# erreur404/Motion-generation-using-quadratic-programs

Hardware: AMD Instinct MI355X
Metric: QP solves/sec at n=7,p=6,m=14 batch=65536; achieved HBM GB/s vs peak (higher is better)
Workload: dtype f64; 1 GPU; C1: 65536 x (n=7, p=6, m=14) general QPs per GPU; kind=general, n=7, p=6, m=14, batch_per_gpu=65536, global_batch=65536, kernel=qp_lane<N=7,M=14>, layout=qp_major, arithmetic=exact: the reference's operation order, bitwise, streams=3, input_sets=5, cold_inputs=True, parallelism=batch-sharded x1

## Files before the change

### motion-generation-using-quadratic-programs_amd/csrc/qp_lane.hip

```cpp
#include <type_traits>
#include <utility>

#include "qp_common.h"

#ifndef QPGPU_LANE_FAST
#define QPGPU_LANE_FAST 0
#endif
#ifndef QPGPU_LANE_UNALIGNED
#define QPGPU_LANE_UNALIGNED 0
#endif
#ifndef QPGPU_LANE_UNIT
#define QPGPU_LANE_UNIT 0
#endif
#if QPGPU_LANE_UNIT && QPGPU_LANE_FAST
#error "the unit-Hessian lane kernels restate the reference's operation order only"
#endif
#if QPGPU_LANE_UNIT && QPGPU_LANE_UNALIGNED
#define QPK_LANE_NS qpk_unit_u
#define QP_LANE_KERNEL qp_lane_unit_kernel
#define QPK_LANE_C(name) name##_unit_u
#elif QPGPU_LANE_UNIT
#define QPK_LANE_NS qpk_unit
#define QP_LANE_KERNEL qp_lane_unit_kernel
#define QPK_LANE_C(name) name##_unit
#elif QPGPU_LANE_FAST && QPGPU_LANE_UNALIGNED
#define QPK_LANE_NS qpk_fast_u
#define QP_LANE_KERNEL qp_lane_fast_kernel
#define QPK_LANE_C(name) name##_fast_u
#elif QPGPU_LANE_FAST
#define QPK_LANE_NS qpk_fast
#define QP_LANE_KERNEL qp_lane_fast_kernel
#define QPK_LANE_C(name) name##_fast
#elif QPGPU_LANE_UNALIGNED
#define QPK_LANE_NS qpk_u
#define QP_LANE_KERNEL qp_lane_kernel
#define QPK_LANE_C(name) name##_u
#else
#define QPK_LANE_NS qpk
#define QP_LANE_KERNEL qp_lane_kernel
#define QPK_LANE_C(name) name
#endif

#ifndef QPGPU_LANE_STAMPS
#define QPGPU_LANE_STAMPS 1
#endif
#if defined(QPGPU_LANE_OCC2) || defined(QPGPU_LANE_DMA_P0) || defined(QPGPU_LANE_CE_LATE) ||       \
    defined(QPGPU_LANE_WARMUP) || defined(QPGPU_LANE_LOOPTOP_EXIT) || defined(QPGPU_LANE_FULL) || \
    defined(QPGPU_LANE_AB_C1ONLY) || defined(QPGPU_LANE_AB_N8P0ONLY)
#error "retired build switch: its default is folded into qp_lane.hip; the other side is an earlier revision (DESIGN 5.15, tools/ab_build.sh SRCFILE=)"
#endif

namespace QPK_LANE_NS {
using namespace qpk;
constexpr bool kFast = QPGPU_LANE_FAST != 0;
constexpr bool kStamps = QPGPU_LANE_STAMPS != 0;
__device__ __forceinline__ void lstamp(const QpArgs& a, int slot) {
  if constexpr (kStamps) qp_stamp(a, slot);
}


struct AgprD {
  uint32_t lo, hi;
};
__device__ __forceinline__ AgprD to_agpr(double v) {
  const uint64_t u = __builtin_bit_cast(uint64_t, v);
  AgprD a;
  asm("v_accvgpr_write_b32 %0, %1" : "=a"(a.lo) : "v"((uint32_t)u));
  asm("v_accvgpr_write_b32 %0, %1" : "=a"(a.hi) : "v"((uint32_t)(u >> 32)));
  return a;
}
__device__ __forceinline__ double from_agpr(const AgprD& a) {
  uint32_t lo, hi;
  asm volatile("v_accvgpr_read_b32 %0, %1" : "=v"(lo) : "a"(a.lo));
  asm volatile("v_accvgpr_read_b32 %0, %1" : "=v"(hi) : "a"(a.hi));
  return __builtin_bit_cast(double, ((uint64_t)hi << 32) | lo);
}

constexpr int kQpw = 64;
constexpr int kLaneOcc = 1;
constexpr int kStage = 5120;
constexpr int kScanDepth = 2;
using LdsD = __attribute__((address_space(3))) double;
using LdsC = __attribute__((address_space(3))) char;
using LdsV = __attribute__((address_space(3))) void;
using GlobalV = __attribute__((address_space(1))) void;
template <int... K, class F>
__device__ __forceinline__ void for_seq_impl(std::integer_sequence<int, K...>, F&& f) {
  (f(std::integral_constant<int, K>{}), ...);
}
template <int N, class F>
__device__ __forceinline__ void for_seq(F&& f) {
  for_seq_impl(std::make_integer_sequence<int, N>{}, f);
}


template <int NM, int MM, int T, bool EXACT, int PX, bool SAFE, bool DUAL = false, bool BOX = false,
          bool FULL = false>
__device__ __forceinline__ bool lane_body(const QpArgs& a, LdsD* lds) {
  double* const sbuf = (double*)lds;
  static_assert(MM <= 64, "bitmask bookkeeping holds m <= 64");
  static_assert(!BOX || (!kFast && MM == 2 * NM), "the box mode is the exact build's, m = 2n");
  static_assert(!FULL || (!kFast && !QPGPU_LANE_UNALIGNED && EXACT && PX >= 0 && !DUAL && !BOX),
                "the full-wave form is the exact aligned build's, for a compile-time shape");
  static_assert(!DUAL || (!kFast && (BOX || (!EXACT && PX < 0))),
                "the dual mode is the exact build's general instantiation, or a box form");
  using RI = RIdx<NM>;
  constexpr int STAGE = kStage;
  constexpr bool F = kFast && !SAFE;
  bool fok = true;
  constexpr bool kLanePrefetch = PX != 0 && !BOX;

  const int lane = threadIdx.x;
  const int64_t b0 = (int64_t)blockIdx.x * kQpw;
  const int64_t b = b0 + lane;
  const int valid = (int)min<int64_t>(kQpw, a.batch - b0);
  const bool live = FULL || lane < valid;

  const int n = EXACT ? NM : a.n;
  const int m = EXACT ? MM : a.m;
  const int p = PX >= 0 ? PX : a.p;
  const double inf = dinf();

#if QPGPU_LANE_UNALIGNED
  const bool full = false;
#else
  const bool full = FULL || (T == 64) || (valid == kQpw);
#endif
  auto copy_chunk = [&](auto J, const double* src, int nd, int off, int k0) {
    constexpr int j = decltype(J)::value;
    static_assert(j >= 0 && j * 1024 < 4096, "the chunk's offset is the instruction's immediate");
    const int e = k0 + 2 * lane;
    __builtin_amdgcn_global_load_lds((const GlobalV*)(e + j * 128 < nd ? src + e : src),
                                     (LdsV*)(lds + off + k0), 16, j * 1024, 0);
  };
  auto copy_run = [&](const double* src, int nd, int off, int k0) {
    copy_chunk(std::integral_constant<int, 0>{}, src, nd, off, k0);
    if (k0 + 128 < nd) copy_chunk(std::integral_constant<int, 1>{}, src, nd, off, k0);
    if (k0 + 256 < nd) copy_chunk(std::integral_constant<int, 2>{}, src, nd, off, k0);
    if (k0 + 384 < nd) copy_chunk(std::integral_constant<int, 3>{}, src, nd, off, k0);
  };
  auto copy_span = [&](const double* src, int nd, int off) {
    if constexpr (FULL) {
#pragma unroll
      for (int k0 = 0; k0 < nd; k0 += 512) copy_run(src, nd, off, k0);
    } else {
#pragma unroll 4
      for (int k = 0; k < nd; k += 128) copy_chunk(std::integral_constant<int, 0>{}, src, nd, off, k);
    }
  };
#if QPGPU_LANE_UNALIGNED
  auto stage_all = [&](const double* X, int E, int off) {
    if constexpr (T == 64) {
      const double* src = X + b0 * (int64_t)E + lane;
      for (int e = 0; e < E; e++) sbuf[off + e * kQpw + lane] = src[e * kQpw];
    } else if (live) {
      const double* src = X + b * (int64_t)E;
      for (int e = 0; e < E; e++) sbuf[off + lane * E + e] = src[e];
    }
  };
  (void)copy_span;
#else
  auto stage_all = [&](const double* X, int E, int off) {
    if (full) {
      copy_span(X + b0 * (int64_t)E, kQpw * E, off);
    } else if (live) {
      const double* src = X + b * (int64_t)E;
      for (int e = 0; e < E; e++) sbuf[off + lane * E + e] = src[e];
    }
  };
#endif
  auto rd_all = [&](int off, int E, int k) -> double {
    if constexpr (T == 64)
      return sbuf[off + k * 64 + lane];
    else
      return sbuf[off + lane * E + k];
  };
  auto view = [&](double* X, int E) -> double* {
    if constexpr (T == 64)
      return X + b0 * (int64_t)E + lane;
    else
      return X + b * (int64_t)E;
  };

  int status = QPGPU_QP_OK;
  double fval = 0.0;
  int iter = 0;
  double xv[NM];
#pragma unroll
  for (int i = 0; i < NM; i++) xv[i] = 0.0;
  double c1 = 0.0, c2 = 0.0;
  constexpr int RB = (STAGE - kQpw * NM) / 2 * 2;
  static_assert(RB >= kQpw * NM * NM, "G and g0 staging exceed the stage buffer");
  constexpr int kCiRowsFit = (RB / kQpw) / MM;
  constexpr int kCiRows = (!BOX && EXACT && T == 1 && MM % 2 == 0) ? (kCiRowsFit < NM ? kCiRowsFit : NM) : 0;
  constexpr bool kCiDma = kCiRows > 0 && PX > 0;
  constexpr int kCeN = PX > 0 ? NM * PX + PX : 1;
  [[maybe_unused]] AgprD ceag[kCiDma ? kCeN : 1];
  const bool dma = kCiDma && (FULL || (a.flags & kArgAligned16));
  double Jreg[NM][NM];
  bool ce_staged = false;
  bool ce_agpr = false;
  constexpr int kPfCI = (NM * MM * 8 + 127) / 128 + 1, kPfC0 = (MM * 8 + 127) / 128 + 1;
  [[maybe_unused]] uint32_t pf[kPfCI + kPfC0];
  bool warmed = false;
  auto warmup = [&]() {
    warmed = true;
    if (live) {
      const int off = dma ? kCiRows * MM * 8 : 0;
      const char* c = reinterpret_cast<const char*>(a.CI + b * (int64_t)(n * m)) + off;
      const char* c0 = reinterpret_cast<const char*>(a.ci0 + b * (int64_t)m);
      const int bc = n * m * 8 - off, b0c = m * 8;
#pragma unroll
      for (int k = 0; k < kPfCI; k++)
        pf[k] = (bc >= 4) ? *reinterpret_cast<const uint32_t*>(c + min(k * 128, bc - 4)) : 0u;
#pragma unroll
      for (int k = 0; k < kPfC0; k++)
        pf[kPfCI + k] = (b0c >= 4) ? *reinterpret_cast<const uint32_t*>(c0 + min(k * 128, b0c - 4)) : 0u;
    }
  };
  constexpr int kCiPieces = kCiRows * MM / 2;
  static_assert(kCiPieces * 16 <= 4096, "the piece's offset is the instruction's immediate");
  auto dma_ci_part = [&](int part, int parts) {
    const int per = (kCiPieces + parts - 1) / parts;
    const double* src = a.CI + (live ? b : b0) * (int64_t)(NM * MM);
    for_seq<kCiPieces>([&](auto K) {
      constexpr int k = decltype(K)::value;
      if (k >= part * per && k < (part + 1) * per)
        __builtin_amdgcn_global_load_lds((const GlobalV*)src, (LdsV*)((LdsC*)lds + k * (kQpw * 16 - 16)), 16,
                                         16 * k, 0);
    });
  };
  lstamp(a, 0);
  [[maybe_unused]] double bv[BOX ? MM : 1];
  if constexpr (BOX) {
    const double* hib = view(const_cast<double*>(a.hi), n);
    const double* lob = view(const_cast<double*>(a.lo), n);
#pragma unroll
    for (int v = 0; v < NM; v++) {
      const double h = (live && v < n) ? hib[v * T] : 0.0;
      const double l = (live && v < n) ? lob[v * T] : 0.0;
      bv[v] = h;
      bv[NM + v] = -l;
    }
  }

  bool chol_ok = live;
  double bad_sum = 0.0;
  {
#if !QPGPU_LANE_UNIT
    double Gr[NM][NM];
#endif
    const int offg0 = RB;
#if !QPGPU_LANE_UNIT
    stage_all(a.G, n * n, 0);
#endif
    stage_all(a.g0, n, offg0);
    __syncthreads();
    double g0v[NM];
#pragma unroll
    for (int i = 0; i < NM; i++) {
#if !QPGPU_LANE_UNIT
#pragma unroll
      for (int j = 0; j < NM; j++) {
        const double v = (i < n && j < n) ? rd_all(0, n * n, i * n + j) : 0.0;
        Gr[i][j] = live ? v : 0.0;
      }
#endif
      const double v0 = i < n ? rd_all(offg0, n, i) : 0.0;
      g0v[i] = live ? v0 : 0.0;
    }
    __syncthreads();
    lstamp(a, 9);
    const int npB = n * p;
    const int offcB = (kQpw * npB + 127) / 128 * 128;
    const bool stageB = p > 0 && offcB + kQpw * p <= STAGE;
    auto round_b = [&](int part) {
      constexpr int parts = NM;
      if (!stageB) return;
      if (!full) {
        if (part == 0) {
          stage_all(a.CE, npB, 0);
          stage_all(a.ce0, p, offcB);
        }
        return;
      }
      const double* ce = a.CE + b0 * (int64_t)npB;
      const double* c0 = a.ce0 + b0 * (int64_t)p;
      if constexpr (EXACT && PX > 0) {
        constexpr int nce = (kQpw * NM * PX + 127) / 128, tot = nce + (kQpw * PX + 127) / 128;
        constexpr int per = (tot + parts - 1) / parts;
        for_seq<tot>([&](auto C) {
          constexpr int c = decltype(C)::value;
          constexpr int arr = c < nce ? 0 : nce;
          constexpr int run = c - c % per > arr ? c - c % per : arr;
          constexpr int j = (c - run) % 4, k0 = (c - j - arr) * 128;
          if (c >= part * per && c < (part + 1) * per) {
            if constexpr (c < nce)
              copy_chunk(std::integral_constant<int, j>{}, ce, kQpw * NM * PX, 0, k0);
            else
              copy_chunk(std::integral_constant<int, j>{}, c0, kQpw * PX, nce * 128, k0);
          }
        });
      } else {
        const int nce = (kQpw * npB + 127) / 128, tot = nce + (kQpw * p + 127) / 128;
        const int per = (tot + parts - 1) / parts;
        for (int c = part * per; c < min(tot, (part + 1) * per); c++) {
          if (c < nce)
            copy_chunk(std::integral_constant<int, 0>{}, ce, kQpw * npB, 0, c * 128);
          else
            copy_chunk(std::integral_constant<int, 0>{}, c0, kQpw * p, offcB, (c - nce) * 128);
        }
      }
    };
#if QPGPU_LANE_UNIT
#pragma unroll
    for (int i = 0; i < NM; i++) {
      round_b(i);
      if (i < n) c1 += 1.0;
    }
#else
#pragma unroll
    for (int i = 0; i < NM; i++)
      if (i < n) c1 += Gr[i][i];
#pragma unroll
    for (int i = 0; i < NM; i++) {
      round_b(i);
      if (i < n && chol_ok) {
        double sum = Gr[i][i];
#pragma unroll
        for (int k = i - 1; k >= 0; k--) sum -= Gr[i][k] * Gr[i][k];
        if (sum <= 0.0) {
          chol_ok = false;
          bad_sum = sum;
        } else {
          const double dg = sqrt(sum);
          Gr[i][i] = dg;
          const double rdg = F ? frcp(dg) : 0.0;
#pragma unroll
          for (int j = i + 1; j < NM; j++)
            if (j < n) {
              double s2 = Gr[i][j];
#pragma unroll
              for (int k = i - 1; k >= 0; k--) s2 -= Gr[i][k] * Gr[j][k];
              Gr[j][i] = ldiv_r<F>(s2, dg, rdg, fok);
            }
#pragma unroll
          for (int k = i + 1; k < NM; k++) Gr[i][k] = Gr[k][i];
        }
      }
    }
    if (!FULL && (a.flags & QPGPU_FLAG_WRITE_FACTOR) && live) {
      double* Gw = view(a.G, n * n);
#pragma unroll
      for (int i = 0; i < NM; i++)
#pragma unroll
        for (int j = 0; j < NM; j++)
          if (i < n && j < n) Gw[(i * n + j) * T] = Gr[i][j];
    }
#endif
    auto land_round_b = [&]() {
    if (p > 0) {
      const int np_ = n * p;
      const int offc = (kQpw * np_ + 127) / 128 * 128;
      ce_staged = offc + kQpw * p <= STAGE;
      __syncthreads();
      lstamp(a, 10);
      if constexpr (kCiDma) {
        if (dma && ce_staged) {
#pragma unroll
          for (int e = 0; e < NM * PX; e++) {
            const double v = rd_all(0, np_, e);
            ceag[e] = to_agpr(live ? v : 0.0);
          }
#pragma unroll
          for (int e = 0; e < PX; e++) {
            const double v = rd_all(offc, p, e);
            ceag[NM * PX + e] = to_agpr(live ? v : 0.0);
          }
          ce_agpr = true;
          __syncthreads();
          lstamp(a, 11);
        }
      }
    }
    };
#if QPGPU_LANE_UNIT
    if (chol_ok) {
#pragma unroll
      for (int r = 0; r < NM; r++) {
#pragma unroll
        for (int j = 0; j < NM; j++) Jreg[r][j] = (r < n && j == r) ? 1.0 : 0.0;
        if (r < n) c2 += 1.0;
      }
#pragma unroll
      for (int i = 0; i < NM; i++) xv[i] = -g0v[i];
#pragma unroll
      for (int i = 0; i < NM; i++)
        if (i < n) fval += g0v[i] * xv[i];
      fval = 0.5 * fval;
    }
#else
    if (chol_ok) {
      bool lfin = true;
#pragma unroll
      for (int i = 0; i < NM; i++)
#pragma unroll
        for (int j = 0; j <= i; j++)
          if (i < n) lfin = lfin && (fabs(Gr[i][j]) < inf);
      double rdiag[NM];
#pragma unroll
      for (int i = 0; i < NM; i++) rdiag[i] = (F && i < n) ? frcp(Gr[i][i]) : 0.0;
      auto build_j = [&](const bool skip) {
#pragma unroll
        for (int r = 0; r < NM; r++) {
          double y[NM];
#pragma unroll
          for (int i = 0; i < NM; i++) {
            double v = 0.0;
            if (r < n && i < n && !(skip && i < r)) {
              v = (i == r) ? 1.0 : 0.0;
#pragma unroll
              for (int j = 0; j < i; j++)
                if (!(skip && j < r)) v -= Gr[i][j] * y[j];
              v = ldiv_r<F>(v, Gr[i][i], rdiag[i], fok);
            }
            y[i] = v;
          }
#pragma unroll
          for (int j = 0; j < NM; j++) Jreg[r][j] = y[j];
          if (r < n) c2 += y[r];
        }
      };
      if (F ? !wave_any(!lfin) : lfin)
        build_j(true);
      else
        build_j(false);
      double y[NM];
#pragma unroll
      for (int i = 0; i < NM; i++) {
        double v = 0.0;
        if (i < n) {
          v = g0v[i];
#pragma unroll
          for (int j = 0; j < i; j++) v -= Gr[i][j] * y[j];
          v = ldiv_r<F>(v, Gr[i][i], rdiag[i], fok);
        }
        y[i] = v;
      }
#pragma unroll
      for (int i = NM - 1; i >= 0; i--) {
        if (i < n) {
          double v = y[i];
#pragma unroll
          for (int j = i + 1; j < NM; j++)
            if (j < n) v -= Gr[i][j] * xv[j];
          xv[i] = ldiv_r<F>(v, Gr[i][i], rdiag[i], fok);
        }
      }
#pragma unroll
      for (int i = 0; i < NM; i++) xv[i] = -xv[i];
#pragma unroll
      for (int i = 0; i < NM; i++)
        if (i < n) fval += g0v[i] * xv[i];
      fval = 0.5 * fval;
    }
#endif
    land_round_b();
  }
  lstamp(a, 1);
  if constexpr (T == 1 && kLanePrefetch) {
    if (!ce_agpr) warmup();
  }
  if (!chol_ok) {
    status = QPGPU_QP_NOT_POSITIVE_DEFINITE;
    fval = bad_sum;
  }
  const bool ok_lane = live && chol_ok;

  double Rv[RI::SIZE];
#pragma unroll
  for (int i = 0; i < RI::SIZE; i++) Rv[i] = 0.0;
  double dv[NM], zv[NM], npv[NM], uv[NM + 1], rv[NM];
  int Av[NM + 1];
#pragma unroll
  for (int i = 0; i < NM; i++) dv[i] = zv[i] = npv[i] = rv[i] = 0.0;
#pragma unroll
  for (int i = 0; i <= NM; i++) {
    uv[i] = 0.0;
    Av[i] = 0;
  }
  double R_norm = 1.0;
  int iq = 0;

  auto compute_d = [&]() {
#pragma unroll
    for (int c = 0; c < NM; c++) {
      double s = 0.0;
#pragma unroll
      for (int j = 0; j < NM; j++)
        if (j < n) s += Jreg[j][c] * npv[j];
      dv[c] = s;
    }
  };
  auto update_z = [&](auto LoC) {
    constexpr int LO = decltype(LoC)::value;
#pragma unroll
    for (int r = 0; r < NM; r++) {
      double z = 0.0;
#pragma unroll
      for (int j = LO; j < NM; j++)
        if (j >= iq && j < n) z += Jreg[r][j] * dv[j];
      zv[r] = z;
    }
  };
  auto update_r = [&](auto LoC) {
    constexpr int LO = decltype(LoC)::value;
#pragma unroll
    for (int i = NM - 1; i >= 0; i--) {
      if (i >= LO && (DUAL || i >= p) && i < iq) {
        double s = 0.0;
#pragma unroll
        for (int j = i + 1; j < NM; j++)
          if (j < iq) s += Rv[RI::at(i, j)] * rv[j];
        rv[i] = ldiv<F>(dv[i] - s, Rv[RI::at(i, i)], fok);
      }
    }
  };
  auto rot_fast = [&](double& a_, double& b_, auto&& apply) {
    const double a0 = a_, b0 = b_;
    const double h = ldistance<true>(a0, b0, fok);
    const bool skip = fabs(h) < kEps;
    const double rh = frcp(h);
    fok = fok && (skip || rcp_ok(rh));
    const bool neg = a0 < 0.0;
    const double cc = fabs(a0) * rh;
    const double ss = (neg ? -b0 : b0) * rh;
    a_ = skip ? a0 : (neg ? -h : h);
    b_ = skip ? b0 : 0.0;
    const double c1_ = skip ? 1.0 : cc, s1_ = skip ? 0.0 : ss;
    const double c2_ = skip ? -1.0 : cc, s2_ = skip ? 0.0 : ss;
    apply([&](double& t1r, double& t2r) {
      const double t1 = t1r, t2 = t2r;
      t1r = c1_ * t1 + s1_ * t2;
      t2r = s2_ * t1 - c2_ * t2;
    });
  };
  auto add_constraint = [&](auto LoC) -> bool {
    constexpr int LO = decltype(LoC)::value;
    if (iq >= n) return false;
#pragma unroll
    for (int j = NM - 1; j >= LO + 1; j--) {
      if (j <= n - 1 && j >= iq + 1) {
        if constexpr (F) {
          rot_fast(dv[j - 1], dv[j], [&](auto&& rot) {
#pragma unroll
            for (int k = 0; k < NM; k++)
              if (k < n) rot(Jreg[k][j - 1], Jreg[k][j]);
          });
          continue;
        }
        double cc = dv[j - 1], ss = dv[j];
        const double h = ldistance<F>(cc, ss, fok);
        if (!(fabs(h) < kEps)) {
          dv[j] = 0.0;
          const double rh = F ? frcp(h) : 0.0;
          ss = ldiv_r<F>(ss, h, rh, fok);
          cc = ldiv_r<F>(cc, h, rh, fok);
          if (cc < 0.0) {
            cc = -cc;
            ss = -ss;
            dv[j - 1] = -h;
          } else {
            dv[j - 1] = h;
          }
          const double xny = ldiv<F>(ss, 1.0 + cc, fok);
#pragma unroll
          for (int k = 0; k < NM; k++)
            if (k < n) {
              const double t1 = Jreg[k][j - 1], t2 = Jreg[k][j];
              const double n1 = t1 * cc + t2 * ss;
              Jreg[k][j - 1] = n1;
              Jreg[k][j] = xny * (t1 + n1) - t2;
            }
        }
      }
    }
    iq++;
#pragma unroll
    for (int c = LO; c < NM; c++)
#pragma unroll
      for (int i = 0; i <= c; i++) {
        const bool w = (c == iq - 1);
        Rv[RI::at(i, c)] = w ? dv[i] : Rv[RI::at(i, c)];
      }
    const double dd = fabs(lsel_lo<LO < NM ? LO : NM - 1>(dv, iq - 1));
    if (dd <= kEps * R_norm) return false;
    R_norm = (R_norm < dd) ? dd : R_norm;
    return true;
  };
  auto delete_constraint = [&](int l, auto LoC) {
    constexpr int LO = decltype(LoC)::value;
    int qq = 0;
    bool found = false;
#pragma unroll
    for (int k = 0; k <= NM; k++)
      if (!found && k >= p && k < iq && Av[k] == l) {
        qq = k;
        found = true;
      }
#pragma unroll
    for (int i = LO; i < NM; i++)
      if (i >= qq && i < iq - 1) {
        Av[i] = Av[i + 1];
        uv[i] = uv[i + 1];
      }
#pragma unroll
    for (int c = LO; c < NM - 1; c++) {
      const bool sh = (c >= qq && c < iq - 1);
#pragma unroll
      for (int r = 0; r <= c + 1 && r < NM; r++) {
        Rv[RI::at(r, c)] = sh ? Rv[RI::at(r, c + 1)] : Rv[RI::at(r, c)];
      }
    }
    {
      const int aiq = lsel_lo<LO>(Av, iq);
      const double uiq = lsel_lo<LO>(uv, iq);
      lput_lo<LO>(Av, iq - 1, aiq);
      lput_lo<LO>(uv, iq - 1, uiq);
      lput_lo<LO>(Av, iq, 0);
      lput_lo<LO>(uv, iq, 0.0);
    }
#pragma unroll
    for (int c = LO; c < NM; c++)
#pragma unroll
      for (int r = 0; r <= c + 1 && r < NM; r++) {
        const bool z = (c == iq - 1) && (r < iq);
        Rv[RI::at(r, c)] = z ? 0.0 : Rv[RI::at(r, c)];
      }
    iq--;
    if (iq == 0) return;
#pragma unroll
    for (int j = LO; j < NM - 1; j++) {
      if (j >= qq && j < iq) {
        if constexpr (F) {
          rot_fast(Rv[RI::at(j, j)], Rv[RI::at(j + 1, j)], [&](auto&& rot) {
#pragma unroll
            for (int k = j + 1; k < NM; k++)
              if (k < iq) rot(Rv[RI::at(j, k)], Rv[RI::at(j + 1, k)]);
#pragma unroll
            for (int k = 0; k < NM; k++)
              if (k < n) rot(Jreg[k][j], Jreg[k][j + 1]);
          });
          continue;
        }
        double cc = Rv[RI::at(j, j)], ss = Rv[RI::at(j + 1, j)];
        const double h = ldistance<F>(cc, ss, fok);
        if (!(fabs(h) < kEps)) {
          const double rh = F ? frcp(h) : 0.0;
          cc = ldiv_r<F>(cc, h, rh, fok);
          ss = ldiv_r<F>(ss, h, rh, fok);
          Rv[RI::at(j + 1, j)] = 0.0;
          if (cc < 0.0) {
            Rv[RI::at(j, j)] = -h;
            cc = -cc;
            ss = -ss;
          } else {
            Rv[RI::at(j, j)] = h;
          }
          const double xny = ldiv<F>(ss, 1.0 + cc, fok);
#pragma unroll
          for (int k = j + 1; k < NM; k++)
            if (k < iq) {
              const double t1 = Rv[RI::at(j, k)], t2 = Rv[RI::at(j + 1, k)];
              const double r1 = t1 * cc + t2 * ss;
              Rv[RI::at(j, k)] = r1;
              Rv[RI::at(j + 1, k)] = xny * (t1 + r1) - t2;
            }
#pragma unroll
          for (int k = 0; k < NM; k++)
            if (k < n) {
              const double t1 = Jreg[k][j], t2 = Jreg[k][j + 1];
              const double n1 = t1 * cc + t2 * ss;
              Jreg[k][j] = n1;
              Jreg[k][j + 1] = xny * (n1 + t1) - t2;
            }
        }
      }
    }
  };
  auto dot = [&](const double(&u_)[NM], const double(&v_)[NM]) -> double {
    double s = 0.0;
#pragma unroll
    for (int i = 0; i < NM; i++)
      if (i < n) s += u_[i] * v_[i];
    return s;
  };
  const auto kZero = std::integral_constant<int, 0>{};
  [[maybe_unused]] auto box_pos = [&](int i) -> int { return i < n ? i : NM + (i - n); };
  [[maybe_unused]] auto compute_d_box = [&](int pos) {
    const bool up = pos < NM;
    const int v = up ? pos : pos - NM;
#pragma unroll
    for (int c = 0; c < NM; c++) {
      double jv = opq_l(Jreg[0][c]);
#pragma unroll
      for (int k = 1; k < NM; k++) jv = (k == v) ? opq_l(Jreg[k][c]) : jv;
      dv[c] = 0.0 + (up ? -jv : jv);
    }
  };

  bool done = !ok_lane;
#pragma unroll
  for (int i = 0; i <= NM; i++) {
    if constexpr (kCiDma) {
      if (ce_agpr && i < PX) dma_ci_part(i, PX);
    }
    if (i < p && !done) {
      iq = i;
      double c0;
      if (i < NM) {
        const int np_ = n * p;
        const int offc = (kQpw * np_ + 127) / 128 * 128;
#pragma unroll
        for (int j = 0; j < NM; j++) {
          if constexpr (kCiDma) {
            if (ce_agpr) {
              npv[j] = j < n ? from_agpr(ceag[(j * PX + i) < kCeN ? j * PX + i : 0]) : 0.0;
              continue;
            }
          }
          if (ce_staged) {
            const double v = j < n ? rd_all(0, np_, j * p + i) : 0.0;
            npv[j] = live ? v : 0.0;
          } else {
            npv[j] = (live && j < n) ? view(const_cast<double*>(a.CE), np_)[(j * p + i) * T] : 0.0;
          }
        }
        bool c0_done = false;
        if constexpr (kCiDma) {
          if (ce_agpr) {
            c0 = from_agpr(ceag[NM * PX + i < kCeN ? NM * PX + i : 0]);
            c0_done = true;
          }
        }
        if (!c0_done) {
          if (ce_staged) {
            const double v = rd_all(offc, p, i);
            c0 = live ? v : 0.0;
          } else {
            c0 = live ? view(const_cast<double*>(a.ce0), p)[i * T] : 0.0;
          }
        }
      } else {
        const double* CEb = view(const_cast<double*>(a.CE), n * p);
#pragma unroll
        for (int j = 0; j < NM; j++) npv[j] = (j < n) ? CEb[(j * p + i) * T] : 0.0;
        c0 = view(const_cast<double*>(a.ce0), p)[i * T];
      }
      compute_d();
      update_z(kZero);
      if constexpr (DUAL) update_r(kZero);
      double t2 = 0.0;
      const double zz = dot(zv, zv);
      const double znp = dot(zv, npv);
      if (fabs(zz) > kEps) t2 = ldiv<F>(-dot(npv, xv) - c0, znp, fok);
#pragma unroll
      for (int k = 0; k < NM; k++) xv[k] += t2 * zv[k];
      uv[i < NM + 1 ? i : NM] = t2;
      if constexpr (DUAL) {
#pragma unroll
        for (int k = 0; k < NM; k++)
          if (k < i) uv[k] -= t2 * rv[k];
      }
      fval += 0.5 * (t2 * t2) * znp;
      Av[i < NM + 1 ? i : NM] = -i - 1;
      if (!add_constraint(kZero)) {
        status = QPGPU_QP_DEPENDENT;
        done = true;
      }
    }
  }
  if (!EXACT && a.x_eq && live) {
    if (chol_ok) {
      double* xb = view(a.x_eq, n);
#pragma unroll
      for (int i = 0; i < NM; i++)
        if (i < n) xb[i * T] = xv[i];
    }
    a.f_eq[b] = fval;
    a.st_eq[b] = status;
  }
  if constexpr (T == 1 && kLanePrefetch) {
    if (live && warmed)
#pragma unroll
      for (int k = 0; k < kPfCI + kPfC0; k++) asm volatile("" ::"v"(pf[k]));
  }
  const bool ci_lds = kCiRows > 0 && (FULL || (a.flags & kArgAligned16));
  bool ci_ready = false;
  if constexpr (kCiDma) {
    if (dma && ce_agpr) {
      __syncthreads();
      ci_ready = true;
    }
  }
  auto ci_lds_at = [&](int e) -> double { return sbuf[((e >> 1) * kQpw + lane) * 2 + (e & 1)]; };
  lstamp(a, 2);
  if constexpr (F) {
    if (wave_any(!fok)) return false;
  }

  constexpr int IQLO = PX >= 0 ? (PX <= NM ? PX : NM) : 0;
  const auto kLo = std::integral_constant<int, IQLO>{};
  constexpr bool kOneFree = FULL && PX >= 0 && PX == NM - 1;
  {
    double sv[MM];
#pragma unroll
    for (int i = 0; i < MM; i++) sv[i] = 0.0;
    double xold[NM], uold[NM];
    int aold[NM];
#pragma unroll
    for (int i = 0; i < NM; i++) {
      xold[i] = uold[i] = 0.0;
      aold[i] = 0;
    }
    uint64_t act = 0;
    uint64_t excl = 0;
    int ip = 0, steps = 0;
    double ss = 0.0, ci0ip = 0.0;
    bool need_scan = true, need_select = true;
    bool active = !done;
    const int max_steps = a.max_steps;
    const double* CIg = view(const_cast<double*>(BOX ? a.g0 : a.CI), n * m);
    const double* ci0g = view(const_cast<double*>(BOX ? a.g0 : a.ci0), m);
    auto uniform_ptr = [](const double* ptr) -> double* {
      const uint64_t v = reinterpret_cast<uint64_t>(ptr);
      const uint32_t lo = __builtin_amdgcn_readfirstlane((uint32_t)v);
      const uint32_t hi = __builtin_amdgcn_readfirstlane((uint32_t)(v >> 32));
      return reinterpret_cast<double*>(((uint64_t)hi << 32) | lo);
    };
    [[maybe_unused]] const auto rsCI = __builtin_amdgcn_make_buffer_rsrc(
        uniform_ptr(BOX ? a.g0 : a.CI + b0 * (int64_t)(n * m)), 0,
        __builtin_amdgcn_readfirstlane(64 * n * m * 8), 0x00020000);
    [[maybe_unused]] const auto rsci0 = __builtin_amdgcn_make_buffer_rsrc(
        uniform_ptr(BOX ? a.g0 : a.ci0 + b0 * (int64_t)m), 0, __builtin_amdgcn_readfirstlane(64 * m * 8),
        0x00020000);
    auto ldCI = [&](int e) -> double {
      if constexpr (T == 64)
        return __builtin_bit_cast(double, __builtin_amdgcn_raw_buffer_load_b64(rsCI, lane * 8, e * 512, 0));
      else
        return CIg[e];
    };
    auto ldci0 = [&](int e) -> double {
      if constexpr (T == 64)
        return __builtin_bit_cast(double, __builtin_amdgcn_raw_buffer_load_b64(rsci0, lane * 8, e * 512, 0));
      else
        return ci0g[e];
    };
    auto lds_pair = [&](int r, int i) -> double2 {
      return *reinterpret_cast<const double2*>(sbuf + (((r * MM + i) >> 1) * kQpw + lane) * 2);
    };
    auto scan_pass = [&]() {
        const bool do_scan = active && need_scan;
        if (wave_any(do_scan)) {
          double psi = 0.0;
          if (do_scan) {
            iter++;
            if constexpr (!kOneFree) {
#pragma unroll
            for (int k = 0; k < NM; k++)
              if (k >= p && k < iq) act |= 1ull << Av[k];
            }
#pragma unroll
            for (int i = 0; i < MM; i++) sv[i] = 0.0;
          }
          if constexpr (BOX) {
            if (do_scan) {
#pragma unroll
              for (int v = 0; v < NM; v++)
                if (v < n) {
                  sv[v] = (0.0 + -xv[v]) + bv[v];
                  sv[NM + v] = (0.0 + xv[v]) + bv[NM + v];
                }
#pragma unroll
              for (int q = 0; q < MM; q++)
                if ((q < NM ? q : q - NM) < n) psi += (sv[q] < 0.0) ? sv[q] : 0.0;
            }
          } else if (do_scan) {
            constexpr bool VEC = (T == 1) && EXACT && (MM % 2 == 0);
            const bool vec = VEC && (FULL || (a.flags & kArgAligned16));
            auto ldrow = [&](double* dst, const double* src) {
              if (VEC && vec) {
#pragma unroll
                for (int i = 0; i < MM; i += 2) {
                  const double2 v = *reinterpret_cast<const double2*>(src + i);
                  dst[i] = v.x;
                  dst[i + 1] = v.y;
                }
              } else {
#pragma unroll
                for (int i = 0; i < MM; i++) dst[i] = (i < m) ? src[i] : 0.0;
              }
            };
            const bool from_chip = ci_lds && ci_ready;
            auto load_row = [&](int r, double* dst) {
              if (r < NM) {
                if (r < n) {
                  if constexpr (T == 1)
                    ldrow(dst, CIg + r * m);
                  else
#pragma unroll
                    for (int i = 0; i < MM; i++) dst[i] = (i < m) ? ldCI(r * m + i) : 0.0;
                }
              } else if (r == NM) {
                if constexpr (T == 1)
                  ldrow(dst, ci0g);
                else
#pragma unroll
                  for (int i = 0; i < MM; i++) dst[i] = (i < m) ? ldci0(i) : 0.0;
              }
            };
            if (kCiRows > 0 && from_chip) {
              constexpr int NG = NM + 1 - kCiRows;
              double gbuf[NG][MM];
#pragma unroll
              for (int r = kCiRows; r <= NM; r++) load_row(r, gbuf[r - kCiRows]);
              __builtin_amdgcn_sched_barrier(0);
#pragma unroll
              for (int j = 0; j < NM; j++) {
                if (j < n) {
                  const double xj = xv[j];
                  if (j < kCiRows) {
#pragma unroll
                    for (int i = 0; i < MM; i += 2) {
                      const double2 v = lds_pair(j, i);
                      if (i < m) sv[i] += v.x * xj;
                      if (i + 1 < m) sv[i + 1] += v.y * xj;
                    }
                  } else {
                    const int g = j - kCiRows < NG ? j - kCiRows : 0;
#pragma unroll
                    for (int i = 0; i < MM; i++)
                      if (i < m) sv[i] += gbuf[g][i] * xj;
                  }
                }
              }
#pragma unroll
              for (int i = 0; i < MM; i++)
                if (i < m) {
                  sv[i] += gbuf[NG - 1][i];
                  psi += (sv[i] < 0.0) ? sv[i] : 0.0;
                }
            } else {
              const bool fill = ci_lds && !ci_ready;
              constexpr int D = kScanDepth;
              double rowbuf[D][MM];
#pragma unroll
              for (int r = 0; r < D - 1; r++) load_row(r, rowbuf[r % D]);
#pragma unroll
              for (int j = 0; j < NM; j++) {
                load_row(j + D - 1, rowbuf[(j + D - 1) % D]);
                __builtin_amdgcn_sched_barrier(0);
                if (j < n) {
                  const double xj = xv[j];
#pragma unroll
                  for (int i = 0; i < MM; i++)
                    if (i < m) sv[i] += rowbuf[j % D][i] * xj;
                  if (j < kCiRows && fill) {
#pragma unroll
                    for (int i = 0; i < MM; i += 2)
                      *reinterpret_cast<double2*>(sbuf + (((j * MM + i) >> 1) * kQpw + lane) * 2) =
                          double2{rowbuf[j % D][i], rowbuf[j % D][i + 1]};
                  }
                }
                __builtin_amdgcn_sched_barrier(0);
              }
#pragma unroll
              for (int i = 0; i < MM; i++)
                if (i < m) {
                  sv[i] += rowbuf[NM % D][i];
                  psi += (sv[i] < 0.0) ? sv[i] : 0.0;
                }
            }
          }
          ci_ready = ci_ready || ci_lds;
          if (do_scan) {
            excl = 0;
            ss = 0.0;
            ip = 0;
            if (fabs(psi) <= (double)m * kEps * c1 * c2 * 100.0) {
              active = false;
            } else if constexpr (!kOneFree) {
#pragma unroll
              for (int i = 0; i < NM; i++) {
                if (i < IQLO || i < iq) {
                  uold[i] = uv[i];
                  aold[i] = Av[i];
                }
                xold[i] = xv[i];
              }
            }
          }
        }
    };
    uint64_t tscan = 0, tsel = 0, nloop = 0, tfirst = 0;
    [[maybe_unused]] uint64_t tdzr = 0, tstep = 0;
    while (wave_any(active)) {
      if constexpr (F) {
        if (wave_any(!fok)) return false;
      }
      const uint64_t tl0 = (kStamps && a.stamps) ? __builtin_amdgcn_s_memtime() : 0;
      scan_pass();
      const uint64_t tl1 = (kStamps && a.stamps) ? __builtin_amdgcn_s_memtime() : 0;
      if (kStamps && a.stamps) {
        tscan += tl1 - tl0;
        if (nloop == 0) tfirst = tl1 - tl0;
      }
      nloop++;
      if constexpr (kOneFree) {
        constexpr int S = NM - 1;
        constexpr int RSS = RI::at(S, S);
        if (active && need_select) {
          const uint32_t blocked = (uint32_t)excl | (iq > S ? 1u << Av[S] : 0u);
#pragma unroll
          for (int i = 0; i < MM; i++) {
            const bool take = sv[i] < ss && !((blocked >> i) & 1u);
            ss = take ? sv[i] : ss;
            ip = take ? i : ip;
          }
          if (ss >= 0.0) {
            active = false;
          } else {
#pragma unroll
            for (int j = 0; j < NM; j++)
              npv[j] = (j < kCiRows && ci_ready) ? ci_lds_at(j * MM + ip) : ldCI(j * m + ip);
#pragma unroll
            for (int i = 0; i < NM; i++) xold[i] = xv[i];
            if (iq == S) uv[S] = 0.0;
          }
        }
        if (kStamps && a.stamps) {
          const double sink = npv[0] + npv[NM - 1];
          asm volatile("" ::"v"(sink));
          tsel += __builtin_amdgcn_s_memtime() - tl1;
        }
        if (active) {
          if (max_steps > 0 && ++steps > max_steps) {
            status = QPGPU_QP_MAX_ITER;
            active = false;
          } else {
            [[maybe_unused]] uint64_t ts0 = 0;
            if constexpr (QPGPU_LANE_STAMPS == 2) ts0 = a.stamps ? __builtin_amdgcn_s_memtime() : 0;
            const bool has = iq > S;
            double dS = 0.0;
#pragma unroll
            for (int j = 0; j < NM; j++) dS += Jreg[j][S] * npv[j];
            double rS = 0.0;
            if (has) {
              rS = ldiv<F>(dS - 0.0, Rv[RSS], fok);
            } else {
#pragma unroll
              for (int r = 0; r < NM; r++) zv[r] = 0.0 + Jreg[r][S] * dS;
            }
            if constexpr (QPGPU_LANE_STAMPS == 2) {
              if (a.stamps) {
                const double sink = rS + zv[0] + dS;
                asm volatile("" ::"v"(sink));
                tdzr += __builtin_amdgcn_s_memtime() - ts0;
              }
            }
            if (has) {
              double t1 = inf;
              if (rS > 0.0) {
                const double q_ = ldiv<F>(uv[S], rS, fok);
                t1 = (q_ < t1) ? q_ : t1;
              }
              if (t1 >= inf) {
                status = QPGPU_QP_INFEASIBLE;
                fval = inf;
                active = false;
              } else {
                uv[S] = 0.0 + t1;
                iq = S;
                need_scan = need_select = false;
              }
            } else {
              const double zz = dot(zv, zv);
              const double znp = dot(zv, npv);
              double t2 = inf;
              if (fabs(zz) > kEps) {
                t2 = ldiv<F>(-ss, znp, fok);
                if (t2 < 0) t2 = inf;
              }
              if (!(t2 < inf)) {
                status = QPGPU_QP_INFEASIBLE;
                fval = inf;
                active = false;
              } else {
                const double t = t2;
#pragma unroll
                for (int k = 0; k < NM; k++) xv[k] += t * zv[k];
                fval += t * znp * (0.5 * t + uv[S]);
                uv[S] = uv[S] + t;
                const double dd = fabs(dS);
                if (dd <= kEps * R_norm) {
                  excl = (uint32_t)excl | (1u << ip);
#pragma unroll
                  for (int i = 0; i < NM; i++) xv[i] = xold[i];
                  need_scan = false;
                  need_select = true;
                } else {
                  R_norm = (R_norm < dd) ? dd : R_norm;
                  Rv[RSS] = dS;
                  Av[S] = ip;
                  iq = S + 1;
                  need_scan = need_select = true;
                }
              }
            }
          }
        }
        continue;
      }
      if (active && need_select) {
        if constexpr (BOX) {
#pragma unroll
          for (int q = 0; q < MM; q++)
            if ((q < NM ? q : q - NM) < n) {
              const int i = q < NM ? q : n + (q - NM);
              const bool elig = !((act >> i) & 1ull) && !((excl >> i) & 1ull);
              const bool take = sv[q] < ss && elig;
              ss = take ? sv[q] : ss;
              ip = take ? i : ip;
            }
        } else {
#pragma unroll
        for (int i = 0; i < MM; i++)
          if (i < m) {
            const bool elig = !((act >> i) & 1ull) && !((excl >> i) & 1ull);
            const bool take = sv[i] < ss && elig;
            ss = take ? sv[i] : ss;
            ip = take ? i : ip;
          }
        }
        if (ss >= 0.0) {
          active = false;
        } else {
          if constexpr (!BOX) {
#pragma unroll
          for (int j = 0; j < NM; j++)
            npv[j] = (j < n) ? ((j < kCiRows && ci_ready) ? ci_lds_at(j * MM + ip) : ldCI(j * m + ip)) : 0.0;
          ci0ip = ldci0(ip);
          }
          lput_lo<IQLO>(uv, iq, 0.0);
          lput_lo<IQLO>(Av, iq, ip);
        }
      }
      if (kStamps && a.stamps) {
        const double sink = npv[0] + ci0ip;
        asm volatile("" ::"v"(sink));
        const uint64_t tl2 = __builtin_amdgcn_s_memtime();
        tsel += tl2 - tl1;
      }
      if (active) {
        if (max_steps > 0 && ++steps > max_steps) {
          status = QPGPU_QP_MAX_ITER;
          active = false;
        } else {
          [[maybe_unused]] uint64_t ts0 = 0;
          if constexpr (QPGPU_LANE_STAMPS == 2) ts0 = a.stamps ? __builtin_amdgcn_s_memtime() : 0;
          [[maybe_unused]] const int ipos = BOX ? box_pos(ip) : ip;
          if constexpr (BOX)
            compute_d_box(ipos);
          else
            compute_d();
          update_z(kLo);
          update_r(kLo);
          if constexpr (QPGPU_LANE_STAMPS == 2) {
            if (a.stamps) {
              const double sink = rv[0] + zv[0] + dv[NM - 1];
              asm volatile("" ::"v"(sink));
              tdzr += __builtin_amdgcn_s_memtime() - ts0;
            }
          }
          int l = 0;
          double t1 = inf;
#pragma unroll
          for (int k = 0; k < NM; k++)
            if (k >= p && k < iq && rv[k] > 0.0) {
              const double q_ = ldiv<F>(uv[k], rv[k], fok);
              const bool take = q_ < t1;
              t1 = take ? q_ : t1;
              l = take ? opq_l(Av[k]) : l;
            }
          const double zz = dot(zv, zv);
          double znp;
          if constexpr (BOX) {
            const double zs = lsel(zv, ipos < NM ? ipos : ipos - NM);
            znp = 0.0 + (ipos < NM ? -zs : zs);
          } else {
            znp = dot(zv, npv);
          }
          double t2;
          if (fabs(zz) > kEps) {
            t2 = ldiv<F>(-lsel<MM>(sv, ipos), znp, fok);
            if (t2 < 0) t2 = inf;
          } else {
            t2 = inf;
          }
          const double t = (t2 < t1) ? t2 : t1;
          const bool infs = t >= inf;
          const bool dual = !infs && t2 >= inf;
          const bool prim = !infs && !dual;
          const bool full = prim && fabs(t - t2) < kEps;
          const bool part = prim && !full;
          if (infs) {
            status = QPGPU_QP_INFEASIBLE;
            fval = inf;
            active = false;
          }
          if (prim) {
#pragma unroll
            for (int k = 0; k < NM; k++) xv[k] += t * zv[k];
            fval += t * znp * (0.5 * t + lsel_lo<IQLO>(uv, iq));
          }
          if (dual || prim) {
#pragma unroll
            for (int k = 0; k < NM; k++)
              if ((DUAL || k >= p) && k < iq) uv[k] -= t * rv[k];
            lput_lo<IQLO>(uv, iq, lsel_lo<IQLO>(uv, iq) + t);
          }
          bool add_fail = false;
          if (full) {
            if (!add_constraint(kLo)) {
              add_fail = true;
              excl |= 1ull << ip;
            } else {
              act |= 1ull << ip;
              need_scan = need_select = true;
            }
          }
          if (dual || part) act &= ~(1ull << l);
          if (dual || part || add_fail) delete_constraint((dual || part) ? l : ip, kLo);
          if (add_fail) {
            act = 0;
#pragma unroll
            for (int i = 0; i < NM; i++)
              if (i >= p && i < iq) {
                Av[i] = aold[i];
                uv[i] = uold[i];
                act |= 1ull << Av[i];
              }
#pragma unroll
            for (int i = 0; i < NM; i++) xv[i] = xold[i];
            need_scan = false;
            need_select = true;
          }
          if (part) {
            if constexpr (BOX) {
              const double xs = lsel(xv, ipos < NM ? ipos : ipos - NM);
              lput_lo<0>(sv, ipos, (0.0 + (ipos < NM ? -xs : xs)) + lsel<MM>(bv, ipos));
            } else {
            double s = 0.0;
#pragma unroll
            for (int j = 0; j < NM; j++)
              if (j < n) s += npv[j] * xv[j];
            lput_lo<0>(sv, ip, s + ci0ip);
            }
          }
          if (dual || part) need_scan = need_select = false;
        }
      }
    }
    if (kStamps && a.stamps && lane == 0) {
      a.stamps[(uint64_t)blockIdx.x * kStampSlots + 5] = tscan;
      a.stamps[(uint64_t)blockIdx.x * kStampSlots + 6] = tsel;
      a.stamps[(uint64_t)blockIdx.x * kStampSlots + 7] = nloop;
      a.stamps[(uint64_t)blockIdx.x * kStampSlots + 8] = tfirst;
      if constexpr (QPGPU_LANE_STAMPS == 2) a.stamps[(uint64_t)blockIdx.x * kStampSlots + 12] = tdzr;
    }
  }
  lstamp(a, 3);
  if constexpr (F) {
    if (wave_any(!fok)) return false;
  }

  if (live) {
    if (chol_ok) {
      double* xb = view(a.x, n);
#pragma unroll
      for (int i = 0; i < NM; i++)
        if (i < n) xb[i * T] = xv[i];
    }
    a.f[b] = fval;
    if (!FULL && a.iters) a.iters[b] = iter;
    a.status[b] = status;
  }
  if constexpr (DUAL) {
    if (live) {
      const bool okq = status == QPGPU_QP_OK;
      double* ub = view(a.u, p + m);
      for (int j = 0; j < p; j++) ub[j * T] = (okq && j <= NM) ? lsel(uv, j) : 0.0;
      double ud[MM];
#pragma unroll
      for (int i = 0; i < MM; i++) ud[i] = 0.0;
#pragma unroll
      for (int k = 0; k < NM; k++) {
        const bool in = okq && k >= p && k < iq;
        const int pos = BOX ? box_pos(Av[k]) : Av[k];
        lput_lo<0>(ud, in ? pos : -1, uv[k]);
      }
      if constexpr (BOX) {
#pragma unroll
        for (int v = 0; v < NM; v++)
          if (v < n) {
            ub[(p + v) * T] = ud[v];
            ub[(p + n + v) * T] = ud[NM + v];
          }
      } else {
#pragma unroll
      for (int i = 0; i < MM; i++)
        if (i < m) ub[(p + i) * T] = ud[i];
      }
      if (a.nact) a.nact[b] = okq ? iq - p : 0;
    }
  }
  lstamp(a, 4);
  return true;
}

template <int NM, int MM, int T, bool EXACT, int PX>
__global__ void __launch_bounds__(64, kLaneOcc) QP_LANE_KERNEL(const QpArgs a) {
  __shared__ double sbuf[kStage];
  if constexpr (kFast) {
    if (!lane_body<NM, MM, T, EXACT, PX, false>(a, (LdsD*)sbuf)) {
      __syncthreads();
      lane_body<NM, MM, T, EXACT, PX, true>(a, (LdsD*)sbuf);
    }
  } else {
    lane_body<NM, MM, T, EXACT, PX, true>(a, (LdsD*)sbuf);
  }
}

#if QPGPU_LANE_UNIT
template <int NM, int MM>
static hipError_t launch_lane_unit(const QpArgs& a, hipStream_t stream) {
  const dim3 g((unsigned)((a.batch + kQpw - 1) / kQpw)), blk(64);
  if (a.tile == 64)
    hipLaunchKernelGGL((QP_LANE_KERNEL<NM, MM, 64, false, -1>), g, blk, 0, stream, a);
  else
    hipLaunchKernelGGL((QP_LANE_KERNEL<NM, MM, 1, false, -1>), g, blk, 0, stream, a);
  return hipGetLastError();
}
}

extern "C" hipError_t QPK_LANE_C(qpk_launch_lane)(const qpk::QpArgs* a, hipStream_t stream) {
  if (a->u || a->hi) return hipErrorInvalidValue;
  if (a->n <= 7 && a->m <= 14) return QPK_LANE_NS::launch_lane_unit<7, 14>(*a, stream);
  if (a->n <= 8 && a->m <= 16) return QPK_LANE_NS::launch_lane_unit<8, 16>(*a, stream);
  return hipErrorInvalidValue;
}
#if !QPGPU_LANE_UNALIGNED
extern "C" const char* QPK_LANE_C(qpk_lane_name)(int n, int m) {
  if (n <= 7 && m <= 14) return "qp_lane_unit<N=7,M=14>";
  if (n <= 8 && m <= 16) return "qp_lane_unit<N=8,M=16>";
  return nullptr;
}
#endif
#else

#if !QPGPU_LANE_FAST && !QPGPU_LANE_UNALIGNED
#define QPK_LANE_HAS_FULL 1
template <int NM, int MM, int T, int PX>
__global__ void __launch_bounds__(64, kLaneOcc) qp_lane_full_kernel(const QpArgs a) {
  __shared__ double sbuf[kStage];
  lane_body<NM, MM, T, true, PX, true, false, false, true>(a, (LdsD*)sbuf);
}
template <int NM, int MM>
static bool full_wave_launch(const QpArgs& a) {
  constexpr uint32_t kAligned = kArgStage16 | kArgAligned16;
  return NM == 7 && MM == 14 && (a.flags & kAligned) == kAligned && !(a.flags & QPGPU_FLAG_WRITE_FACTOR) &&
         !a.iters;
}
#else
#define QPK_LANE_HAS_FULL 0
template <int NM, int MM>
static bool full_wave_launch(const QpArgs&) {
  return false;
}
#endif
template <class Full, class Rest>
static void launch_full_then_rest(const QpArgs& a, Full&& full, Rest&& rest) {
  const int64_t nb = a.batch / kQpw, done = nb * kQpw;
  if (nb > 0) {
    QpArgs c = a;
    c.batch = done;
    full(c, dim3((unsigned)nb));
    qpk_lane_count_launch(1);
  }
  if (a.batch > done) {
    QpArgs c = sub_range(a, done, a.batch - done);
    c.stamps = a.stamps ? a.stamps + nb * kStampSlots : nullptr;
    rest(c, dim3(1));
    qpk_lane_count_launch(0);
  }
}

#ifndef QPGPU_LANE_PART
#define QPGPU_LANE_PART 0
#endif
#if !QPGPU_LANE_FAST && QPGPU_LANE_PART != 2
template <int NM, int MM, int T>
__global__ void __launch_bounds__(64, kLaneOcc) qp_lane_dual_kernel(const QpArgs a) {
  __shared__ double sbuf[kStage];
  lane_body<NM, MM, T, false, -1, true, true>(a, (LdsD*)sbuf);
}
template <int NM, int MM, int T, bool EXACT, int PX>
__global__ void __launch_bounds__(64, kLaneOcc) qp_lane_box_kernel(const QpArgs a) {
  __shared__ double sbuf[kStage];
  lane_body<NM, MM, T, EXACT, PX, true, false, true>(a, (LdsD*)sbuf);
}
template <int NM, int MM, int T, bool EXACT, int PX>
__global__ void __launch_bounds__(64, kLaneOcc) qp_lane_box_dual_kernel(const QpArgs a) {
  __shared__ double sbuf[kStage];
  lane_body<NM, MM, T, EXACT, PX, true, true, true>(a, (LdsD*)sbuf);
}
#endif
template <int NM, int MM, int T>
static hipError_t launch_lane_p0(const QpArgs& a, hipStream_t stream);
template <int NM, int MM, int T>
static hipError_t launch_lane_t(const QpArgs& a, hipStream_t stream) {
  const int64_t blocks = (a.batch + kQpw - 1) / kQpw;
  const dim3 g((unsigned)blocks), blk(64);
  switch (mode_of(a)) {
#if !QPGPU_LANE_FAST && QPGPU_LANE_PART != 2
    case kBoxDual:
    case kBox:
      if (a.m != 2 * a.n || a.x_eq) return hipErrorInvalidValue;
      if (a.u) {
        if (a.n == NM && a.p == 0)
          hipLaunchKernelGGL((qp_lane_box_dual_kernel<NM, MM, T, true, 0>), g, blk, 0, stream, a);
        else
          hipLaunchKernelGGL((qp_lane_box_dual_kernel<NM, MM, T, false, -1>), g, blk, 0, stream, a);
      } else if (a.n == NM && a.p == 0) {
        hipLaunchKernelGGL((qp_lane_box_kernel<NM, MM, T, true, 0>), g, blk, 0, stream, a);
      } else {
        hipLaunchKernelGGL((qp_lane_box_kernel<NM, MM, T, false, -1>), g, blk, 0, stream, a);
      }
      return hipSuccess;
    case kDual:
      hipLaunchKernelGGL((qp_lane_dual_kernel<NM, MM, T>), g, blk, 0, stream, a);
      return hipSuccess;
#else
    case kBoxDual:
    case kBox:
    case kDual:
      return hipErrorInvalidValue;
#endif
    case kPlain:
      break;
  }
  if (a.n == NM && a.m == MM && !a.x_eq) {
#if QPK_LANE_HAS_FULL
    if constexpr (NM == 7 && MM == 14)
      if (a.p == 6 && full_wave_launch<NM, MM>(a)) {
        launch_full_then_rest(
            a,
            [&](const QpArgs& c, dim3 gc) {
              hipLaunchKernelGGL((qp_lane_full_kernel<NM, MM, T, 6>), gc, blk, 0, stream, c);
            },
            [&](const QpArgs& c, dim3 gc) {
              hipLaunchKernelGGL((QP_LANE_KERNEL<NM, MM, T, true, 6>), gc, blk, 0, stream, c);
            });
        return hipSuccess;
      }
#endif
    if (a.p == 6)
      hipLaunchKernelGGL((QP_LANE_KERNEL<NM, MM, T, true, 6>), g, blk, 0, stream, a);
    else if (a.p == 0)
      return launch_lane_p0<NM, MM, T>(a, stream);
    else
      hipLaunchKernelGGL((QP_LANE_KERNEL<NM, MM, T, true, -1>), g, blk, 0, stream, a);
  } else {
    hipLaunchKernelGGL((QP_LANE_KERNEL<NM, MM, T, false, -1>), g, blk, 0, stream, a);
  }
  return hipSuccess;
}

#if QPGPU_LANE_PART == 1
}
extern "C" hipError_t qpk_launch_lane_p0(const qpk::QpArgs* a, hipStream_t stream);
namespace QPK_LANE_NS {
template <int NM, int MM, int T>
static hipError_t launch_lane_p0(const QpArgs& a, hipStream_t stream) {
  return qpk_launch_lane_p0(&a, stream);
}
#else
template <int NM, int MM, int T>
static hipError_t launch_lane_p0(const QpArgs& a, hipStream_t stream) {
#if QPK_LANE_HAS_FULL
  if constexpr (NM == 7 && MM == 14)
    if (full_wave_launch<NM, MM>(a)) {
      launch_full_then_rest(
          a,
          [&](const QpArgs& c, dim3 gc) {
            hipLaunchKernelGGL((qp_lane_full_kernel<NM, MM, T, 0>), gc, dim3(64), 0, stream, c);
          },
          [&](const QpArgs& c, dim3 gc) {
            hipLaunchKernelGGL((QP_LANE_KERNEL<NM, MM, T, true, 0>), gc, dim3(64), 0, stream, c);
          });
      return hipSuccess;
    }
#endif
  const int64_t blocks = (a.batch + kQpw - 1) / kQpw;
  hipLaunchKernelGGL((QP_LANE_KERNEL<NM, MM, T, true, 0>), dim3((unsigned)blocks), dim3(64), 0, stream, a);
  return hipSuccess;
}
#endif

#if QPGPU_LANE_PART != 2
template <int NM, int MM>
static hipError_t launch_lane(const QpArgs& a, hipStream_t stream) {
  const hipError_t e = a.tile == 64 ? launch_lane_t<NM, MM, 64>(a, stream) : launch_lane_t<NM, MM, 1>(a, stream);
  if (e != hipSuccess) return e;
  return hipGetLastError();
}

struct LaneVariant {
  int nmax, mmax;
  const char* name[4];
  hipError_t (*launch)(const QpArgs&, hipStream_t);
};

#if QPGPU_LANE_FAST
#define QPK_LANE_NAMES(s) {"qp_lane_fast<" s ">", nullptr, nullptr, nullptr}
#else
#define QPK_LANE_NAMES(s) {"qp_lane<" s ">", "qp_lane_dual<" s ">", "qp_lane_box<" s ">", "qp_lane_box_dual<" s ">"}
#endif
static const LaneVariant kLaneVariants[] = {
    {7, 14, QPK_LANE_NAMES("N=7,M=14"), launch_lane<7, 14>},
    {8, 16, QPK_LANE_NAMES("N=8,M=16"), launch_lane<8, 16>},
};

const LaneVariant* pick_lane(int n, int m) {
  for (const auto& v : kLaneVariants)
    if (n <= v.nmax && m <= v.mmax) return &v;
  return nullptr;
}
#endif

}

#if QPGPU_LANE_PART == 2
extern "C" hipError_t qpk_launch_lane_p0(const qpk::QpArgs* a, hipStream_t stream) {
  using namespace QPK_LANE_NS;
  if (a->n == 7 && a->m == 14)
    return a->tile == 64 ? launch_lane_p0<7, 14, 64>(*a, stream) : launch_lane_p0<7, 14, 1>(*a, stream);
  if (a->n == 8 && a->m == 16)
    return a->tile == 64 ? launch_lane_p0<8, 16, 64>(*a, stream) : launch_lane_p0<8, 16, 1>(*a, stream);
  return hipErrorInvalidValue;
}
#else
extern "C" hipError_t QPK_LANE_C(qpk_launch_lane)(const qpk::QpArgs* a, hipStream_t stream) {
  const QPK_LANE_NS::LaneVariant* v = QPK_LANE_NS::pick_lane(a->n, a->m);
  return v ? v->launch(*a, stream) : hipErrorInvalidValue;
}
#if !QPGPU_LANE_UNALIGNED
extern "C" const char* QPK_LANE_C(qpk_lane_name)(int n, int m, int mode) {
  const QPK_LANE_NS::LaneVariant* v = QPK_LANE_NS::pick_lane(n, m);
  return v ? v->name[mode] : nullptr;
}
#endif
#endif
#endif
```

Measured before the change: 2.357 billion QP solves/s.

## Keep non-DMA constraint rows and ci0 register-resident across scan passes

In the one-free-variable DMA path, the constraint-matrix rows not covered by the LDS copy, plus ci0, are loaded once into registers (ci0 and xold in AGPRs). Each later scan reads them from registers instead of reloading from global memory. The selection step also picks the new column from the kept rows, which removes the per-iteration global loads for those rows. This raises register pressure (VGPR/AGPR), which may lower occupancy or cause spills. The scan is restructured into a helper that runs at the end of each loop iteration instead of at the start.

```diff
diff --git a/motion-generation-using-quadratic-programs_amd/csrc/qp_lane.hip b/motion-generation-using-quadratic-programs_amd/csrc/qp_lane.hip
--- a/motion-generation-using-quadratic-programs_amd/csrc/qp_lane.hip
+++ b/motion-generation-using-quadratic-programs_amd/csrc/qp_lane.hip
@@ -93,6 +93,91 @@
   for_seq_impl(std::make_integer_sequence<int, N>{}, f);
 }
 
+
+template <bool ON, int ROWS, int NM, int MM>
+struct LaneResident {
+  double kept[ROWS][MM];
+  AgprD ci0_ag[MM], xold_ag[NM];
+};
+template <int ROWS, int NM, int MM>
+struct LaneResident<false, ROWS, NM, MM> {
+  char kept, ci0_ag, xold_ag;
+};
+
+template <int NM, int MM, int ROWS, bool LOAD>
+__device__ __forceinline__ void lane_scan_kept(const double* sbuf, int lane, const double* CIg, const double* ci0g,
+                                               const double (&xv)[NM], double (&kept)[NM - ROWS][MM],
+                                               AgprD (&ci0_ag)[MM], double (&sv)[MM], double c1, double c2,
+                                               bool need_scan, bool& active, int& iter, uint64_t& excl, double& ss,
+                                               int& ip) {
+  const bool do_scan = active && need_scan;
+  if (!wave_any(do_scan)) return;
+  if (do_scan) {
+    iter++;
+    double c0[MM];
+    if constexpr (LOAD) {
+#pragma unroll
+      for (int r = ROWS; r <= NM; r++) {
+        const double* src = r < NM ? CIg + r * MM : ci0g;
+#pragma unroll
+        for (int i = 0; i < MM; i += 2) {
+          const double2 v = *reinterpret_cast<const double2*>(src + i);
+          (r < NM ? kept[r < NM ? r - ROWS : 0][i] : c0[i]) = v.x;
+          (r < NM ? kept[r < NM ? r - ROWS : 0][i + 1] : c0[i + 1]) = v.y;
+        }
+      }
+      __builtin_amdgcn_sched_barrier(0);
+    }
+#pragma unroll
+    for (int i = 0; i < MM; i++) sv[i] = 0.0;
+    constexpr int AHEAD = LOAD ? 0 : 1;
+    double2 row[2][MM / 2];
+    auto ldrow = [&](int j, double2(&dst)[MM / 2]) {
+#pragma unroll
+      for (int i = 0; i < MM; i += 2)
+        dst[i / 2] = *reinterpret_cast<const double2*>(sbuf + (((j * MM + i) >> 1) * kQpw + lane) * 2);
+    };
+#pragma unroll
+    for (int j = 0; j < AHEAD; j++) ldrow(j, row[j % 2]);
+#pragma unroll
+    for (int j = 0; j < NM; j++) {
+      const double xj = xv[j];
+      if (j + AHEAD < ROWS) ldrow(j + AHEAD, row[(j + AHEAD) % 2]);
+      if constexpr (!LOAD) {
+        if (j == ROWS) {
+#pragma unroll
+          for (int i = 0; i < MM; i++) c0[i] = from_agpr(ci0_ag[i]);
+        }
+      }
+      __builtin_amdgcn_sched_barrier(0);
+      if (j < ROWS) {
+#pragma unroll
+        for (int i = 0; i < MM; i += 2) {
+          sv[i] += row[j % 2][i / 2].x * xj;
+          sv[i + 1] += row[j % 2][i / 2].y * xj;
+        }
+      } else {
+#pragma unroll
+        for (int i = 0; i < MM; i++) sv[i] += kept[j >= ROWS ? j - ROWS : 0][i] * xj;
+      }
+      __builtin_amdgcn_sched_barrier(0);
+    }
+    double psi = 0.0;
+#pragma unroll
+    for (int i = 0; i < MM; i++) {
+      sv[i] += c0[i];
+      psi += (sv[i] < 0.0) ? sv[i] : 0.0;
+    }
+    if constexpr (LOAD) {
+#pragma unroll
+      for (int i = 0; i < MM; i++) ci0_ag[i] = to_agpr(c0[i]);
+    }
+    excl = 0;
+    ss = 0.0;
+    ip = 0;
+    if (fabs(psi) <= (double)MM * kEps * c1 * c2 * 100.0) active = false;
+  }
+}
 
 template <int NM, int MM, int T, bool EXACT, int PX, bool SAFE, bool DUAL = false, bool BOX = false,
           bool FULL = false>
@@ -1004,18 +1089,37 @@
     };
     uint64_t tscan = 0, tsel = 0, nloop = 0, tfirst = 0;
     [[maybe_unused]] uint64_t tdzr = 0, tstep = 0;
+    constexpr bool kResident = kOneFree && kCiDma;
+    constexpr int kKept = kResident ? NM - kCiRows : 1;
+    static_assert(!kResident || (kQpw * NM * PX + 127) / 128 * 128 + kQpw * PX <= STAGE,
+                  "the kept-row scan reads the LDS copy the DMA path fills");
+    [[maybe_unused]] LaneResident<kResident, kKept, NM, MM> res;
+    [[maybe_unused]] auto& kept = res.kept;
+    [[maybe_unused]] auto& ci0_ag = res.ci0_ag;
+    [[maybe_unused]] auto& xold_ag = res.xold_ag;
+    if constexpr (kResident) {
+      const uint64_t ts0 = (kStamps && a.stamps) ? __builtin_amdgcn_s_memtime() : 0;
+      if (kStamps && a.stamps && wave_any(active)) nloop = 1;
+      lane_scan_kept<NM, MM, kCiRows, true>(sbuf, lane, CIg, ci0g, xv, kept, ci0_ag, sv, c1, c2, need_scan, active,
+                                            iter, excl, ss, ip);
+      if (kStamps && a.stamps) tfirst = tscan = __builtin_amdgcn_s_memtime() - ts0;
+#pragma unroll
+      for (int i = 0; i < NM; i++) xold_ag[i] = to_agpr(xv[i]);
+    }
     while (wave_any(active)) {
       if constexpr (F) {
         if (wave_any(!fok)) return false;
       }
       const uint64_t tl0 = (kStamps && a.stamps) ? __builtin_amdgcn_s_memtime() : 0;
-      scan_pass();
-      const uint64_t tl1 = (kStamps && a.stamps) ? __builtin_amdgcn_s_memtime() : 0;
-      if (kStamps && a.stamps) {
-        tscan += tl1 - tl0;
-        if (nloop == 0) tfirst = tl1 - tl0;
-      }
-      nloop++;
+      if constexpr (!kResident) scan_pass();
+      const uint64_t tl1 = kResident ? tl0 : (kStamps && a.stamps) ? __builtin_amdgcn_s_memtime() : 0;
+      if constexpr (!kResident) {
+        if (kStamps && a.stamps) {
+          tscan += tl1 - tl0;
+          if (nloop == 0) tfirst = tl1 - tl0;
+        }
+        nloop++;
+      }
       if constexpr (kOneFree) {
         constexpr int S = NM - 1;
         constexpr int RSS = RI::at(S, S);
@@ -1026,15 +1130,24 @@
             const bool take = sv[i] < ss && !((blocked >> i) & 1u);
             ss = take ? sv[i] : ss;
             ip = take ? i : ip;
+            if constexpr (kResident) {
+#pragma unroll
+              for (int j = kCiRows; j < NM; j++) npv[j] = take ? kept[j - kCiRows < kKept ? j - kCiRows : 0][i] : npv[j];
+            }
           }
           if (ss >= 0.0) {
             active = false;
           } else {
 #pragma unroll
-            for (int j = 0; j < NM; j++)
+            for (int j = 0; j < (kResident ? kCiRows : NM); j++)
               npv[j] = (j < kCiRows && ci_ready) ? ci_lds_at(j * MM + ip) : ldCI(j * m + ip);
 #pragma unroll
-            for (int i = 0; i < NM; i++) xold[i] = xv[i];
+            for (int i = 0; i < NM; i++) {
+              if constexpr (kResident)
+                xold_ag[i] = to_agpr(xv[i]);
+              else
+                xold[i] = xv[i];
+            }
             if (iq == S) uv[S] = 0.0;
           }
         }
@@ -1105,7 +1218,12 @@
                 if (dd <= kEps * R_norm) {
                   excl = (uint32_t)excl | (1u << ip);
 #pragma unroll
-                  for (int i = 0; i < NM; i++) xv[i] = xold[i];
+                  for (int i = 0; i < NM; i++) {
+                    if constexpr (kResident)
+                      xv[i] = from_agpr(xold_ag[i]);
+                    else
+                      xv[i] = xold[i];
+                  }
                   need_scan = false;
                   need_select = true;
                 } else {
@@ -1118,6 +1236,13 @@
               }
             }
           }
+        }
+        if constexpr (kResident) {
+          const uint64_t ts0 = (kStamps && a.stamps) ? __builtin_amdgcn_s_memtime() : 0;
+          if (kStamps && a.stamps && wave_any(active)) nloop++;
+          lane_scan_kept<NM, MM, kCiRows, false>(sbuf, lane, CIg, ci0g, xv, kept, ci0_ag, sv, c1, c2, need_scan,
+                                                 active, iter, excl, ss, ip);
+          if (kStamps && a.stamps) tscan += __builtin_amdgcn_s_memtime() - ts0;
         }
         continue;
       }
```

After: 2.509 billion QP solves/s, median of 6. 1.06x the previous value.
